# qdrvm/erasure-coding-crust

Hardware: AMD Instinct MI355X
Metric: device-resident encode+reconstruct GiB/s (and % HBM roofline), n_val=1024 (higher is better)
Workload: dtype u16

## Files before the change

### erasure-coding-crust_amd/csrc/capi.cpp

```cpp
#include <hip/hip_runtime.h>

#include <algorithm>
#include <chrono>
#include <cstdio>
#include <cstdlib>
#include <cstring>
#include <optional>
#include <string>
#include <vector>

#include "../../include/erasure_coding/ec_amd.h"
#include "../../include/erasure_coding/erasure_coding.h"
#include "ec_kernels.hpp"
#include "ec_runtime.hpp"
#include "gf_field.hpp"

using namespace ecamd;

namespace {

struct Workspace {
  void *ptr;
  size_t bytes;
};
// ... 568 lines not shown
                                      unsigned long slen, unsigned long sstride,
                                      const uint8_t *d_present, const uint16_t *d_err_log,
                                      unsigned long batch, uint8_t *d_out,
                                      unsigned long ostride, void *stream) {
  return ECCR_AMD_reconstruct_batch_patterns(nv, d_shards, slen, sstride, d_present, d_err_log,
                                             nullptr, batch, d_out, ostride, stream);
}

const char *ECCR_AMD_encode_kernel(unsigned long nv, const uint8_t *d_payloads, unsigned long plen,
                                   unsigned long pstride, unsigned long batch,
                                   const uint8_t *d_shards, unsigned long sstride) {
  CodeParams p;
  if (code_params(nv, &p) != ParamError::kOk || plen == 0) return nullptr;
  if (sstride < shard_len(p.k, plen) || pstride < plen) return nullptr;
  return kernel_name(choose_encode(p, plen, pstride, batch, reinterpret_cast<uintptr_t>(d_payloads),
                                   reinterpret_cast<uintptr_t>(d_shards), sstride));
}

const char *ECCR_AMD_reconstruct_kernel(unsigned long nv, const uint8_t *d_shards,
                                        unsigned long slen, unsigned long sstride,
                                        const uint8_t *d_present, const uint16_t *d_err_log,
                                        unsigned long batch, const uint8_t *d_out,
                                        unsigned long ostride) {
  CodeParams p;
  if (code_params(nv, &p) != ParamError::kOk || slen % 2 != 0) return nullptr;
  if (sstride < slen || ostride < slen * p.k) return nullptr;
  const ReconOverrides &o = recon_overrides();
  return kernel_name(choose_reconstruct(
      p, slen, sstride, batch, reinterpret_cast<uintptr_t>(d_shards),
      reinterpret_cast<uintptr_t>(d_present), reinterpret_cast<uintptr_t>(d_err_log),
      reinterpret_cast<uintptr_t>(d_out), ostride, o.waves8, o.force_packed));
}

NPRSResult ECCR_AMD_locator_cache_stats(unsigned long *hits, unsigned long *misses) {
  DeviceState *d = device_state();
  if (!d) return result(NPRS_RESULT_UNKNOWN_RECONSTRUCTION);
  locator_cache_stats(d, hits, misses);
  return result(NPRS_RESULT_OK);
}

NPRSResult ECCR_AMD_systematic_batch(unsigned long nv, const uint8_t *d_shards, unsigned long slen,
                                     unsigned long sstride, unsigned long batch, uint8_t *d_out,
                                     unsigned long ostride, void *stream) {
  CodeParams p;
  NPRSResult r = params_or_error(nv, &p);
  if (r.tag != NPRS_RESULT_OK) return r;
  if (sstride < slen || ostride < slen / 2 * 2 * p.k) return result(NPRS_RESULT_NON_UNIFORM_CHUNKS);
  if (!device_state()) return result(NPRS_RESULT_UNKNOWN_RECONSTRUCTION);
  if (!hip_check(launch_systematic(p, d_shards, slen / 2 * 2, sstride, batch, d_out, ostride,
                                   static_cast<hipStream_t>(stream)),
                 "systematic launch"))
    return result(NPRS_RESULT_UNKNOWN_RECONSTRUCTION);
  return result(NPRS_RESULT_OK);
}

void ECCR_AMD_set_scratch_limit(unsigned long bytes) { set_scratch_limit(bytes); }

int ECCR_AMD_release_stream_scratch(void *stream) {
  DeviceState *d = device_state();
  return d && release_stream_scratch(d, static_cast<hipStream_t>(stream)) ? 1 : 0;
}

const char *ECCR_AMD_last_error(void) { return last_error(); }

}
```

### erasure-coding-crust_amd/csrc/dec_n1024x.hip

```cpp
#include <hip/hip_runtime.h>

#include "dec_n1024_common.hpp"
#include "ec_device.hpp"
#include "ec_kernels.hpp"
#include "cimg.hpp"

namespace ecamd {
namespace {
using namespace n1024;
constexpr int WAVES = 12;
constexpr int THREADS = 64 * WAVES;
constexpr int COLS = 4 * WAVES;
constexpr int TAB_REGION = int(kCImgBytes);
static_assert(TAB_REGION % 8192 == 0, "regions 8 KB aligned: region addresses are base | rz");
constexpr uint32_t STG = uint32_t(TAB_REGION + WAVES * REG_BYTES);
constexpr uint32_t STG_PITCH = 112;
__device__ __forceinline__ uint32_t stg_row(uint32_t y) { return STG + (((y & 3) << 6) | (y >> 2)) * STG_PITCH; }
constexpr uint32_t SLOT = STG + 256 * STG_PITCH;
constexpr int LDS_BYTES = int(SLOT + 16);
static_assert(LDS_BYTES <= 160 * 1024, "LDS budget");
constexpr int ROW_WORDS = COLS / 2;

__host__ __device__ constexpr uint32_t rz(uint32_t v) {
  return ((v >> 5) << 8) | (((v ^ (v >> 4) ^ (v >> 5)) & 31) << 3);
}

__device__ __forceinline__ uint32_t posA2_reg(int r) { return uint32_t(r & 3) | (uint32_t(r >> 2) << 8); }
__device__ __forceinline__ uint32_t posB2_lane(uint32_t lane) { return (lane & 3) | ((lane >> 2) << 6); }
__device__ __forceinline__ uint32_t posC_reg(int r) {
  return (uint32_t((r >> 2) & 3) << 6) | (uint32_t(r & 3) << 8);
}

__device__ __forceinline__ void ipassA2(S16 &s, uint32_t lane) {
  const uint32_t l0 = cimg_lin(lane << 1), l1 = cimg_lin(lane);
  SubTab S0, S1;
  F9Tab F0, F1;
  Tab G0, G1;
  ctab(l0, cimg_lin(0), S0);
  ctab(l0, cimg_lin(1), S1);
  ctab(l0, cimg_lin(128), F0);
  ib(s, 0, 1, S0);
  ctab(l0, cimg_lin(129), F1);
  ib(s, 2, 3, S1);
  ctab(l0, cimg_lin(256), G0);
  ib(s, 4, 5, F0);
  ctab(l0, cimg_lin(257), G1);
  ib(s, 6, 7, F1);
  ib(s, 8, 9, G0);
  ctab(l0, cimg_lin(384), G0);
  ib(s, 10, 11, G1);
  ctab(l0, cimg_lin(385), G1);
  ctab(l1, cimg_lin(0), S0);
  ib(s, 12, 13, G0);
  ctab(l1, cimg_lin(64), S1);
// ... 42 lines not shown
  ctab(0u, cimg_lin(3), X3);
  ctab(0u, cimg_lin(4), X4);
  bx(s, 0, 4);
  ib(s, 8, 12, X1);
  ib(s, 1, 5, X2);
  ib(s, 9, 13, X3);
  ib(s, 2, 6, X4);
  ctab(0u, cimg_lin(5), X4);
  ib(s, 10, 14, X4);
  ctab(0u, cimg_lin(6), X4);
  ib(s, 3, 7, X4);
  ctab(0u, cimg_lin(7), X4);
  ib(s, 11, 15, X4);
  bx(s, 0, 8);
  bx(s, 4, 12);
  ib(s, 1, 9, X1);
  ib(s, 5, 13, X1);
  ib(s, 2, 10, X2);
  ib(s, 6, 14, X2);
  ib(s, 3, 11, X3);
  ib(s, 7, 15, X3);
#pragma unroll
  for (int q = 0; q < 4; ++q) {
    bx(s, 4 * q, 4 * q + 1);
    ib(s, 4 * q + 2, 4 * q + 3, X1);
  }
#pragma unroll
  for (int q = 0; q < 4; ++q) {
    bx(s, 4 * q, 4 * q + 2);
    bx(s, 4 * q + 1, 4 * q + 3);
  }
}

__device__ __forceinline__ void load_row_tail96(const uint8_t *row, uint32_t avail, uint32_t (&w)[ROW_WORDS]) {
  const uint32_t nw = (avail + 3) / 4;
  const uint32_t last = (avail & 3) ? (1u << (8 * (avail & 3))) - 1 : ~0u;
  const uint32_t *r = reinterpret_cast<const uint32_t *>(row);
#pragma unroll
  for (int j = 0; j < ROW_WORDS; ++j) {
    w[j] = 0;
    if (uint32_t(j) < nw) w[j] = r[j] & (uint32_t(j) + 1 == nw ? last : ~0u);
  }
}

}

__global__ void __launch_bounds__(THREADS) reconstruct_n1024x(
    const uint8_t *__restrict__ shards, uint64_t slen, uint64_t sstride,
    const uint8_t *__restrict__ present, const uint16_t *__restrict__ elog,
    const uint32_t *__restrict__ pattern, const uint32_t *__restrict__ order,
    uint8_t *__restrict__ out, uint64_t ostride, int nv, uint32_t batch, uint32_t *tick, DevTables t) {
  extern __shared__ __attribute__((aligned(16))) uint8_t lds[];
  uint8_t *regions = lds + TAB_REGION;
  volatile uint32_t *slot = reinterpret_cast<volatile uint32_t *>(lds + SLOT);
  const uint32_t tid0 = threadIdx.x, wave = tid0 >> 6;
  uint32_t taken = 0;
  if (tid0 == 0) taken = gridDim.x + atomicAdd(tick, 1u);
  uint8_t *my = regions + wave * REG_BYTES;

  {
    constexpr int kPer = (TAB_REGION / 16 + THREADS - 1) / THREADS;
    typedef uint32_t v4u __attribute__((ext_vector_type(4)));
    v4u v[kPer];
#pragma unroll
    for (int k = 0; k < kPer; ++k) {
      const uint32_t i = tid0 + k * THREADS;
      if (i < uint32_t(TAB_REGION / 16)) v[k] = reinterpret_cast<const v4u *>(t.cimg)[i];
    }
#pragma unroll
    for (int k = 0; k < kPer; ++k) {
      const uint32_t i = tid0 + k * THREADS;
      if (i < uint32_t(TAB_REGION / 16)) reinterpret_cast<v4u *>(lds)[i] = v[k];
    }
  }
  __syncthreads();
  if (tid0 == 0) *slot = taken;

  const uint64_t ncols = slen / 2;
  const uint32_t tiles_pp = uint32_t((ncols + COLS - 1) / COLS);
  const uint64_t total = uint64_t(tiles_pp) * batch;
  const uint32_t wave_s = __builtin_amdgcn_readfirstlane(tid0 >> 6);
  const auto load_meta = [&](uint64_t bw, uint32_t tid, uint32_t (&m)[4]) {
    const uint64_t pt = pattern ? pattern[bw] : bw;
    m[0] = order[bw * N + tid];
    m[1] = tid + THREADS < uint32_t(N) ? order[bw * N + THREADS + tid] : 0xFFFFu;
    const uint32_t y0 = 4 * (tid & 63);
    const uint32_t p4 = *reinterpret_cast<const uint32_t *>(present + pt * N + y0);
    const uint2 e4 = *reinterpret_cast<const uint2 *>(elog + pt * N + y0);
#pragma unroll
    for (int q = 0; q < 4; ++q) {
      const uint32_t e = ((q < 2 ? e4.x : e4.y) >> (16 * (q & 1))) & 0xFFFFu;
      const uint32_t f = ((p4 >> (8 * q)) & 0xFFu) ? 0xFFFFu : mul_index(e);
      if (q & 1) m[2 + (q >> 1)] |= f << 16;
      else m[2 + (q >> 1)] = f;
    }
  };
  uint32_t meta[4] = {0, 0, 0, 0}, meta_next[4] = {0, 0, 0, 0};
  uint32_t cur = blockIdx.x;
  if (cur < total) load_meta(cur / tiles_pp, tid0, meta);
  while (cur < total) {
    uint32_t tid = tid0;
    asm volatile("" : "+v"(tid));
    const uint32_t lane = tid & 63;
    const uint32_t bq = cur / tiles_pp;
    const uint64_t b = bq, col0 = uint64_t(cur - bq * tiles_pp) * COLS;
    const uint8_t *SH = shards + b * uint64_t(nv) * sstride;
    uint8_t *O = out + b * ostride;

    uint32_t nxt;
    {
      uint32_t w[ROW_WORDS] = {};
      Tab RT = {};
      const uint64_t avail = slen - 2 * col0;
      const auto load_row = [&](int half) __attribute__((always_inline)) {
        const uint8_t *row = SH + uint64_t(meta[half] >> 16) * sstride + 2 * col0;
        if (avail >= 2 * COLS) {
#pragma unroll
          for (int q = 0; q < ROW_WORDS / 4; ++q) {
            const uint4 d = reinterpret_cast<const uint4 *>(row)[q];
            w[4 * q] = d.x;
            w[4 * q + 1] = d.y;
            w[4 * q + 2] = d.z;
            w[4 * q + 3] = d.w;
          }
        } else {
          load_row_tail96(row, uint32_t(avail), w);
        }
        load_tab(t.mtab_tin, meta[half] & 0xffffu, RT);
      };
      if ((meta[0] & 0xffffu) != 0xffffu) load_row(0);
      lds_barrier();
      nxt = __builtin_amdgcn_readfirstlane(*slot);
      if (tid0 == 0) taken = gridDim.x + atomicAdd(tick, 1u);
#pragma unroll
      for (int half = 0; half < 2; ++half) {
        if (half == 1 && tid >= uint32_t(N - THREADS)) break;
        const uint32_t v = meta[half] >> 16;
        const bool on = (meta[half] & 0xffffu) != 0xffffu;
        if (half == 1 && on) load_row(1);
        uint32_t l[WAVES], h[WAVES];
#pragma unroll
        for (int g = 0; g < WAVES; ++g) l[g] = h[g] = 0;
        if (on) {
          if (v < uint32_t(K)) {
#pragma unroll
            for (int j = 0; j < ROW_WORDS / 4; ++j)
              *reinterpret_cast<__attribute__((address_space(3))) v4u *>(uintptr_t(stg_row(v) + 16 * j)) =
                  v4u{w[4 * j], w[4 * j + 1], w[4 * j + 2], w[4 * j + 3]};
          }
#pragma unroll
          for (int g = 0; g < WAVES; ++g) {
            const uint32_t a = w[2 * g], c = w[2 * g + 1];
            const uint32_t xh = vperm(c, a, 0x06040200u), xl = vperm(c, a, 0x07050301u);
            mul_acc(xl, xh, RT, l[g], h[g]);
          }
        }
#pragma unroll
        for (int g = 0; g < WAVES; ++g)
          *reinterpret_cast<uint2 *>(regions + g * REG_BYTES + rz(v)) = make_uint2(l[g], h[g]);
      }
    }
    if (nxt < total) load_meta(nxt / tiles_pp, tid, meta_next);
    __syncthreads();
    const uint64_t cbase = col0 + 4 * uint64_t(wave_s);
    if (cbase >= ncols) {
#pragma unroll
      for (int i = 0; i < 4; ++i) meta[i] = meta_next[i];
      cur = nxt;
      continue;
    }

    S16 s;
    {
      const uint32_t la = lds_addr(my) | rz(lane << 2);
#pragma unroll
      for (int r = 0; r < 16; ++r) {
        const uint2 x = lds_ld2(la ^ rz(posA2_reg(r)));
        s.l[r] = x.x;
        s.h[r] = x.y;
      }
      ipassA2(s, lane);
#pragma unroll
      for (int r = 0; r < 16; ++r) lds_st2(la ^ rz(posA2_reg(r)), make_uint2(s.l[r], s.h[r]));
      __builtin_amdgcn_fence(__ATOMIC_ACQ_REL, "wavefront");
      __builtin_amdgcn_wave_barrier();
    }
    {
      const uint32_t lb = lds_addr(my) | rz(posB2_lane(lane));
#pragma unroll
      for (int r = 0; r < 16; ++r) {
        const uint2 x = lds_ld2(lb ^ rz(uint32_t(r) << 2));
        s.l[r] = x.x;
        s.h[r] = x.y;
      }
      ipassB2(s, lane);
#pragma unroll
      for (int r = 0; r < 16; ++r) lds_st2(lb ^ rz(uint32_t(r) << 2), make_uint2(s.l[r], s.h[r]));
      __builtin_amdgcn_fence(__ATOMIC_ACQ_REL, "wavefront");
      __builtin_amdgcn_wave_barrier();
    }
    const uint32_t lc = lds_addr(my) | rz(lane);
#pragma unroll
    for (int r = 0; r < 16; ++r) {
      const uint2 x = lds_ld2(lc ^ rz(posC_reg(r)));
      s.l[r] = x.x;
      s.h[r] = x.y;
    }
    ipassC2(s);

    Tab T5[4];
#pragma unroll
    for (int q = 0; q < 4; ++q) {
      const uint32_t m = (meta[2 + (q >> 1)] >> (16 * (q & 1))) & 0xFFFFu;
      load_tab(t.mtab_tout, m != 0xFFFFu ? m : 0u, T5[q]);
    }

    uint32_t ql[4], qh[4];
    {
      const uint32_t keep0 = ((lane ^ (lane >> 1)) & 1) ? 0u : 0xffffffffu;
      const uint32_t m4 = ((lane >> 4) & 1) ? 0u : 0xffffffffu;
      const uint32_t m5 = ((lane >> 5) & 1) ? 0u : 0xffffffffu;
      const auto lane_terms = [&](uint32_t c0, uint32_t acc) {
        acc ^= uint32_t(__builtin_amdgcn_update_dpp(0, int(c0), 0xF5, 0xf, 0xf, false));
        acc ^= uint32_t(__builtin_amdgcn_update_dpp(0, int(c0), 0xEE, 0xf, 0xf, false));
        acc ^= uint32_t(__builtin_amdgcn_update_dpp(0, int(c0), 0x104, 0xf, 0x5, false));
        acc ^= uint32_t(__builtin_amdgcn_update_dpp(0, int(c0), 0x108, 0xf, 0x3, false));
        acc = __builtin_amdgcn_bitop3_b32(acc, from_upper(c0, 4), m4, 0x78);
        acc = __builtin_amdgcn_bitop3_b32(acc, from_upper(c0, 5), m5, 0x78);
        return __builtin_amdgcn_bitop3_b32(acc, c0, keep0, 0x78);
      };
#pragma unroll
      for (int q = 0; q < 4; ++q) {
        uint32_t al = s.l[4 * q + 1] ^ s.l[4 * q + 2], ah = s.h[4 * q + 1] ^ s.h[4 * q + 2];
        if (!(q & 1)) {
          al ^= s.l[4 * (q | 1)];
          ah ^= s.h[4 * (q | 1)];
        }
        if (!(q & 2)) {
          al ^= s.l[4 * (q | 2)];
          ah ^= s.h[4 * (q | 2)];
        }
        ql[q] = lane_terms(s.l[4 * q], al);
// ... 61 lines not shown
      swap_bit(qh[1], qh[3], 3, l3);
      fb(0, 2, T[0]);
      fb(1, 3, T[0]);
      ctab(0u, L(8), T[0]);
      fb(0, 1, T[1]);
      ctab(0u, L(9), T[1]);
      fb(2, 3, T[0]);
      ctab(0u, L(10), T[0]);
      const bool l0 = lane & 1, l1 = (lane >> 1) & 1;
      swap_bit(ql[0], ql[1], 0, l0);
      swap_bit(qh[0], qh[1], 0, l0);
      swap_bit(ql[2], ql[3], 0, l0);
      swap_bit(qh[2], qh[3], 0, l0);
      swap_bit(ql[0], ql[2], 1, l1);
      swap_bit(qh[0], qh[2], 1, l1);
      swap_bit(ql[1], ql[3], 1, l1);
      swap_bit(qh[1], qh[3], 1, l1);
      fb(0, 2, T[1]);
      fb(1, 3, T[1]);
      ctab(0u, L(11), T[1]);
      fb(0, 1, T[0]);
      fb(2, 3, T[1]);
    }

    {
      uint32_t ol[4], oh[4];
#pragma unroll
      for (int q = 0; q < 4; ++q) {
        const uint32_t m = (meta[2 + (q >> 1)] >> (16 * (q & 1))) & 0xFFFFu;
        ol[q] = oh[q] = 0;
        if (m != 0xFFFFu) {
          mul_acc(ql[q], qh[q], T5[q], ol[q], oh[q]);
        } else {
          const uint2 rv = lds_ld2(stg_row(4 * lane + uint32_t(q)) + 8 * wave_s);
          oh[q] = vperm(rv.y, rv.x, 0x06040200u);
          ol[q] = vperm(rv.y, rv.x, 0x07050301u);
        }
      }
#pragma unroll
      for (int c = 0; c < 4; ++c) {
        const uint64_t col = cbase + c;
        if (col >= ncols) break;
        const uint32_t w0 = vperm(ol[0], oh[0], 0x0c0c0400u + 0x0101u * c) |
                            (vperm(ol[1], oh[1], 0x0c0c0400u + 0x0101u * c) << 16);
        const uint32_t w1 = vperm(ol[2], oh[2], 0x0c0c0400u + 0x0101u * c) |
                            (vperm(ol[3], oh[3], 0x0c0c0400u + 0x0101u * c) << 16);
        *reinterpret_cast<uint2 *>(O + (col * K + 4 * lane) * 2) = make_uint2(w0, w1);
      }
    }
    if (tid0 == 0) *slot = taken;
#pragma unroll
    for (int i = 0; i < 4; ++i) meta[i] = meta_next[i];
    cur = nxt;
  }
}

size_t n1024_tick_offset(const CodeParams &p, size_t batch) { return (gather_order_bytes(p, batch) + 255) / 256 * 256; }
size_t n1024_scratch_bytes(const CodeParams &p, size_t batch) { return n1024_tick_offset(p, batch) + 256; }

static_assert(size_t(COLS) == kN1024xMinCols, "choose_reconstruct: at least one whole tile");

hipError_t launch_reconstruct_n1024x(const CodeParams &p, const DevTables &t,
                                     const uint8_t *d_shards, size_t slen, size_t sstride,
                                     const uint8_t *d_present, const uint16_t *d_err_log,
                                     const uint32_t *d_pattern, size_t batch, uint8_t *d_out,
                                     size_t ostride, void *scratch, hipStream_t s) {
  int cus = 0;
  if (!t.cimg || !scratch || slen / 2 < size_t(COLS)) return hipErrorInvalidValue;
  if (const hipError_t e = prepare_kernel(reinterpret_cast<const void *>(&reconstruct_n1024x), LDS_BYTES, &cus);
      e != hipSuccess)
    return e;
  const size_t tiles = (slen / 2 + COLS - 1) / COLS * batch;
  if (tiles + 4096 >= (size_t(1) << 32)) return hipErrorInvalidValue;
  uint32_t *order = static_cast<uint32_t *>(scratch);
  uint32_t *tick = reinterpret_cast<uint32_t *>(static_cast<uint8_t *>(scratch) + n1024_tick_offset(p, batch));
  if (const hipError_t e = launch_gather_order(p, d_present, d_err_log, d_pattern, batch, order, s);
      e != hipSuccess)
    return e;
  if (const hipError_t e = launch_zero_counters(tick, sizeof(uint32_t), s); e != hipSuccess) return e;
  const unsigned grid = unsigned(tiles < size_t(cus) ? tiles : size_t(cus));
  hipLaunchKernelGGL(reconstruct_n1024x, dim3(grid), dim3(THREADS), LDS_BYTES, s, d_shards, uint64_t(slen),
                     uint64_t(sstride), d_present, d_err_log, d_pattern, order, d_out, uint64_t(ostride),
                     int(p.nv), uint32_t(batch), tick, t);
  return hipGetLastError();
}

}
```

### erasure-coding-crust_amd/csrc/ec_kernels.hip

```cpp
#include <hip/hip_runtime.h>

#include <cstdlib>

#include "ec_device.hpp"
#include "ec_kernels.hpp"

namespace ecamd {
namespace {

constexpr int kBlock = 256;
constexpr int kLdsSlots = 4096;

__device__ __forceinline__ void ld(uint2 *p, uint32_t &l, uint32_t &h) {
  const uint2 v = *p;
  l = v.x;
  h = v.y;
}

constexpr int kPreStages = 3;
__device__ void ifft_g(uint2 *S, int logG, int logsz, uint32_t index, const DevTables t) {
  const int G = 1 << logG;
  const int half = (1 << logsz) >> 1;
  if (logsz <= kPreStages && half * G <= int(blockDim.x)) {
    const int b = threadIdx.x, g = b & (G - 1), pi = b >> logG;
// ... 609 lines not shown
  const size_t shm = size_t(p.n) * sizeof(uint16_t);
  int cus = 0;
  if (const hipError_t e = prepare_kernel(reinterpret_cast<const void *>(&error_locator_g), 65536 * 2, &cus);
      e != hipSuccess)
    return e;
  hipLaunchKernelGGL(error_locator_g, dim3(unsigned(batch)), dim3(kBlock), shm, s, d_present,
                     int(p.nv), ilog2(p.n), d_fold, d_pattern, d_err_log,
                     static_cast<uint16_t *>(nullptr));
  return hipGetLastError();
}

hipError_t launch_broadcast_locators(const CodeParams &p, const uint32_t *d_pattern, size_t batch,
                                     uint16_t *d_err_log, hipStream_t s) {
  if (batch == 0) return hipSuccess;
  hipLaunchKernelGGL(pattern_broadcast, dim3(unsigned(batch)), dim3(kBlock), 0, s, d_pattern,
                     int(p.n), d_err_log);
  return hipGetLastError();
}

size_t reconstruct_scratch_bytes(const CodeParams &p, size_t slen, size_t batch) {
  if (n4096_applicable(p)) return n4096_scratch_bytes(p, batch);
  if (n1024_applicable(p)) return n1024_scratch_bytes(p, batch);
  if (decgen_applicable(p)) return gather_order_bytes(p, batch);
  if (p.n <= uint32_t(kLdsSlots)) return 0;
  const size_t tiles = (slen / 2 + 3) / 4;
  return tiles * grid_y(batch) * 2 * size_t(p.n) * sizeof(uint2);
}

const ReconOverrides &recon_overrides() {
  static const ReconOverrides o = [] {
    const char *w = std::getenv("ECCR_AMD_RECON_WAVES"), *k = std::getenv("ECCR_AMD_RECON_PACKED");
    ReconOverrides r;
    r.waves8 = w && w[0] == '8';
    r.force_packed = k && k[0] == '1';
    return r;
  }();
  return o;
}

Kernel choose_reconstruct(const CodeParams &p, size_t slen, size_t sstride, size_t batch,
                          uintptr_t shards, uintptr_t present, uintptr_t err_log, uintptr_t out,
                          size_t ostride, bool waves8, bool force_packed) {
  if (batch == 0 || slen < 2) return Kernel::invalid;
  const bool aligned = shards % 16 == 0 && out % 8 == 0 && sstride % 16 == 0 &&
                       (batch == 1 || ostride % 8 == 0);
  const bool out8 = out % 8 == 0 && (batch == 1 || ostride % 8 == 0) && present % 16 == 0 &&
                    err_log % 16 == 0;
  const bool out16 = out % 16 == 0 && (batch == 1 || ostride % 16 == 0);
  const size_t ncols = slen / 2;
  if (n1024_applicable(p)) {
    const bool packed = ncols < kN1024Cols || shards % 16 != 0 || sstride % 16 != 0;
    if (!packed && aligned && out8 && !waves8 && ncols >= kN1024xMinCols) return Kernel::reconstruct_n1024x;
    if (packed ? out8 && shards % 2 == 0 && sstride % 2 == 0 : aligned && out8) {
      if (!packed && !force_packed) return Kernel::reconstruct_n1024;
      const size_t ncols4 = (ncols + 3) / 4 * 4;
      return ncols4 * batch + kN1024Cols < (size_t(1) << 32) ? Kernel::reconstruct_n1024_packed
                                                             : Kernel::invalid;
    }
  }
  if (aligned && out16 && n4096_applicable(p)) return Kernel::reconstruct_n4096;
  if (aligned && out16 && decgen_applicable(p)) return Kernel::reconstruct_gen;
  return Kernel::reconstruct_g;
}

hipError_t launch_reconstruct(const CodeParams &p, const DevTables &t, const uint8_t *d_shards,
                              size_t slen, size_t sstride, const uint8_t *d_present,
// ... 55 lines not shown
```

### erasure-coding-crust_amd/csrc/ec_kernels.hpp

```cpp
#pragma once

#include <hip/hip_runtime.h>

#include <cstddef>
#include <cstdint>

#include "gf_field.hpp"

namespace ecamd {

constexpr size_t kTabImageBytes = 5 * 1024 * 16;
constexpr int kTabImages = 4;

constexpr int tower_sub_min(int q) { return q == 0 ? 2 : q == 1 ? 3 : 4; }

constexpr int kF9Images = 2;
constexpr bool f9_slot(int kind, uint32_t i) {
  return i % 4 == 1 || (kind == 1 && i % 2 == 0 && i >= 256 && i < 512);
}

constexpr uint32_t kCImgGen = 0, kCImgGenPlane = 4096;
constexpr uint32_t kCImgF9 = 20480, kCImgF9Plane = 2048;
constexpr uint32_t kCImgSub0 = 28672, kCImgSub1 = 30720;
constexpr uint32_t kCImgBytes = 32768;
// ... 22 lines not shown

struct HostSig {
  uint32_t *flag = nullptr;
  uint32_t v = 0;
  bool fused = false;
};

hipError_t prepare_kernel(const void *fn, int lds_bytes, int *cus);

size_t encode_scratch_bytes(const CodeParams &p, size_t payload_len, size_t batch);
bool encode_scratch_optional(const CodeParams &p);
size_t reconstruct_scratch_bytes(const CodeParams &p, size_t shard_len, size_t batch);

enum class Kernel {
  invalid,
  encode_k256w,
  encode_k256_packed,
  encode_kw,
  encode_k512w,
  encode_k1024,
  encode_g,
  reconstruct_n1024x,
  reconstruct_n1024,
  reconstruct_n1024_packed,
  reconstruct_n4096,
  reconstruct_gen,
  reconstruct_g,
};
const char *kernel_name(Kernel k);

Kernel choose_encode(const CodeParams &p, size_t payload_len, size_t payload_stride, size_t batch,
                     uintptr_t payloads, uintptr_t shards, size_t shard_stride);
struct ReconOverrides {
  bool waves8 = false, force_packed = false;
};
const ReconOverrides &recon_overrides();
Kernel choose_reconstruct(const CodeParams &p, size_t shard_len, size_t shard_stride, size_t batch,
                          uintptr_t shards, uintptr_t present, uintptr_t err_log, uintptr_t out,
                          size_t out_stride, bool waves8, bool force_packed);

hipError_t launch_encode(const CodeParams &p, const DevTables &t, const uint8_t *d_payloads,
                         size_t payload_len, size_t payload_stride, size_t batch, uint8_t *d_shards,
                         size_t shard_stride, void *scratch, hipStream_t s, HostSig *sig = nullptr);

hipError_t launch_error_locator(const CodeParams &p, const uint8_t *d_present, size_t batch,
                                const uint16_t *d_fold, const uint32_t *d_pattern,
                                uint16_t *d_err_log, hipStream_t s);
bool locator_wave_applicable(uint32_t n);
hipError_t launch_signal_host(uint32_t *h_flag, uint32_t v, hipStream_t s);
hipError_t launch_zero_counters(uint32_t *p, size_t bytes, hipStream_t s);
size_t dedup_scratch_bytes(size_t batch);
hipError_t launch_dedup_patterns(const CodeParams &p, const uint8_t *d_present, size_t batch,
                                 uint32_t *d_pattern, void *scratch, hipStream_t s);
hipError_t launch_broadcast_locators(const CodeParams &p, const uint32_t *d_pattern, size_t batch,
                                     uint16_t *d_err_log, hipStream_t s);

hipError_t launch_reconstruct(const CodeParams &p, const DevTables &t, const uint8_t *d_shards,
                              size_t shard_len, size_t shard_stride, const uint8_t *d_present,
                              const uint16_t *d_err_log, const uint32_t *d_pattern, size_t batch,
                              uint8_t *d_out, size_t out_stride, void *scratch, hipStream_t s);

hipError_t launch_systematic(const CodeParams &p, const uint8_t *d_shards, size_t shard_len,
                             size_t shard_stride, size_t batch, uint8_t *d_out, size_t out_stride,
                             hipStream_t s, HostSig *sig = nullptr);

constexpr int kTinyMaxN = 16;
constexpr size_t kTinyBytes = 2048;
bool tiny_applicable(const CodeParams &p, size_t plen, size_t ostride);
hipError_t launch_encode_tiny(const CodeParams &p, const DevTables &t, const uint8_t *h_payload, size_t plen,
                              uint8_t *out, size_t ostride, hipStream_t s, HostSig *sig);
bool systematic_tiny_applicable(const CodeParams &p, size_t slen);
hipError_t launch_systematic_tiny(const CodeParams &p, const uint8_t *h_shards, size_t slen, size_t sstride,
                                  uint8_t *out, hipStream_t s, HostSig *sig);
hipError_t warm_encode_tiny(hipStream_t s);

bool k256_applicable(const CodeParams &p);
constexpr size_t kK256Tile = 128, kN1024Cols = 32, kN1024xMinCols = 48;
hipError_t launch_encode_k256(const CodeParams &p, const DevTables &t, const uint8_t *d_payloads,
                              size_t plen, size_t pstride, size_t batch, uint8_t *d_shards,
                              size_t sstride, hipStream_t s);
size_t k256_scratch_bytes(const CodeParams &p);
hipError_t launch_encode_k256w(const CodeParams &p, const DevTables &t, const uint8_t *d_payloads,
                               size_t plen, size_t pstride, size_t batch, uint8_t *d_shards,
                               size_t sstride, void *scratch, hipStream_t s);

bool k1024_applicable(const CodeParams &p);
size_t k1024_scratch_bytes(size_t plen, size_t batch);
hipError_t launch_encode_k1024(const CodeParams &p, const DevTables &t, const uint8_t *d_payloads,
                               size_t plen, size_t pstride, size_t batch, uint8_t *d_shards,
                               size_t sstride, void *scratch, hipStream_t s);

bool k512w_applicable(const CodeParams &p);
size_t k512w_scratch_bytes(const CodeParams &p);
hipError_t launch_encode_k512w(const CodeParams &p, const DevTables &t, const uint8_t *d_payloads,
                               size_t plen, size_t pstride, size_t batch, uint8_t *d_shards,
                               size_t sstride, void *scratch, hipStream_t s);

bool kw_applicable(const CodeParams &p);
size_t kw_scratch_bytes(const CodeParams &p);
hipError_t launch_encode_kw(const CodeParams &p, const DevTables &t, const uint8_t *d_payloads,
                            size_t plen, size_t pstride, size_t batch, uint8_t *d_shards,
                            size_t sstride, void *scratch, hipStream_t s);

size_t gather_order_bytes(const CodeParams &p, size_t batch);
hipError_t launch_gather_order(const CodeParams &p, const uint8_t *d_present,
                               const uint16_t *d_err_log, const uint32_t *d_pattern, size_t batch,
                               uint32_t *order, hipStream_t s);

bool n1024_applicable(const CodeParams &p);
hipError_t launch_reconstruct_n1024(const CodeParams &p, const DevTables &t, bool packed,
                                    const uint8_t *d_shards, size_t slen, size_t sstride,
                                    const uint8_t *d_present, const uint16_t *d_err_log,
                                    const uint32_t *d_pattern, size_t batch, uint8_t *d_out,
                                    size_t ostride, void *scratch, hipStream_t s);
size_t n1024_scratch_bytes(const CodeParams &p, size_t batch);
size_t n1024_tick_offset(const CodeParams &p, size_t batch);
hipError_t launch_reconstruct_n1024x(const CodeParams &p, const DevTables &t,
                                     const uint8_t *d_shards, size_t slen, size_t sstride,
                                     const uint8_t *d_present, const uint16_t *d_err_log,
                                     const uint32_t *d_pattern, size_t batch, uint8_t *d_out,
                                     size_t ostride, void *scratch, hipStream_t s);

bool n4096_applicable(const CodeParams &p);
size_t n4096_scratch_bytes(const CodeParams &p, size_t batch);
hipError_t launch_reconstruct_n4096(const CodeParams &p, const DevTables &t,
                                    const uint8_t *d_shards, size_t slen, size_t sstride,
                                    const uint8_t *d_present, const uint16_t *d_err_log,
                                    const uint32_t *d_pattern, size_t batch, uint8_t *d_out,
                                    size_t ostride, void *scratch, hipStream_t s);

bool decgen_applicable(const CodeParams &p);
hipError_t launch_reconstruct_gen(const CodeParams &p, const DevTables &t,
                                  const uint8_t *d_shards, size_t slen, size_t sstride,
                                  const uint8_t *d_present, const uint16_t *d_err_log,
                                  const uint32_t *d_pattern, size_t batch, uint8_t *d_out,
                                  size_t ostride, void *scratch, hipStream_t s);

}
```

### erasure-coding-crust_amd/ecc_amd.py

```python
from __future__ import annotations

import ctypes as C
import enum
import os
import subprocess

try:
    import torch
except Exception:
    torch = None

HERE = os.path.dirname(os.path.abspath(__file__))
LIB_PATH = os.environ.get("ECC_AMD_LIB") or os.path.join(HERE, "lib", "liberasure_coding_crust.so")
HEADERS = [os.path.join(os.path.dirname(HERE), "include", "erasure_coding", h)
           for h in ("erasure_coding.h", "ec_amd.h")]


class Tag(enum.IntEnum):
    OK = 0
    TOO_MANY_VALIDATORS = 1
    NOT_ENOUGH_VALIDATORS = 2
    WRONG_VALIDATOR_COUNT = 3
    NOT_ENOUGH_CHUNKS = 4
    TOO_MANY_CHUNKS = 5
# ... 53 lines not shown

def lib():
    global _lib
    if _lib is None:
        if not os.path.exists(LIB_PATH):
            build()
        L = C.CDLL(LIB_PATH)
        ul, up, vp = C.c_ulong, C.POINTER(C.c_ulong), C.c_void_p
        sig = {
            "ECCR_get_recovery_threshold": (NPRSResult, [ul, up]),
            "ECCR_deallocate_data_block": (None, [C.POINTER(DataBlock)]),
            "ECCR_deallocate_chunk": (None, [C.POINTER(Chunk)]),
            "ECCR_deallocate_chunk_list": (None, [C.POINTER(ChunksList)]),
            "ECCR_AFFT_Table": (NPRSResult, [C.POINTER(C.c_uint16 * 65535)]),
            "ECCR_Test_MeasurePerformance": (NPRSResult, [C.POINTER(DataBlock), ul, up, up]),
            "ECCR_obtain_chunks": (NPRSResult, [ul, C.POINTER(DataBlock), C.POINTER(ChunksList)]),
            "ECCR_reconstruct_from_systematic": (NPRSResult, [ul, C.POINTER(ChunksList),
                                                              C.POINTER(DataBlock)]),
            "ECCR_reconstruct": (NPRSResult, [ul, C.POINTER(ChunksList), C.POINTER(DataBlock)]),
            "ECCR_AMD_code_params": (NPRSResult, [ul, up, up, up]),
            "ECCR_AMD_shard_len": (ul, [ul, ul]),
            "ECCR_AMD_device_count": (C.c_int, []),
            "ECCR_AMD_init_device": (NPRSResult, []),
            "ECCR_AMD_encode_batch": (NPRSResult, [ul, vp, ul, ul, ul, vp, ul, vp]),
            "ECCR_AMD_error_locator": (NPRSResult, [ul, vp, ul, vp, vp]),
            "ECCR_AMD_reconstruct_batch": (NPRSResult, [ul, vp, ul, ul, vp, vp, ul, vp, ul, vp]),
            "ECCR_AMD_systematic_batch": (NPRSResult, [ul, vp, ul, ul, ul, vp, ul, vp]),
            "ECCR_AMD_dedup_patterns": (NPRSResult, [ul, vp, ul, vp, vp]),
            "ECCR_AMD_error_locator_patterns": (NPRSResult, [ul, vp, vp, ul, vp, vp]),
            "ECCR_AMD_reconstruct_batch_patterns": (NPRSResult, [ul, vp, ul, ul, vp, vp, vp, ul, vp,
                                                                 ul, vp]),
            "ECCR_AMD_encode_kernel": (C.c_char_p, [ul, vp, ul, ul, ul, vp, ul]),
            "ECCR_AMD_reconstruct_kernel": (C.c_char_p, [ul, vp, ul, ul, vp, vp, ul, vp, ul]),
            "ECCR_AMD_locator_cache_stats": (NPRSResult, [up, up]),
            "ECCR_AMD_encode_workspace_bytes": (ul, [ul, ul, ul]),
            "ECCR_AMD_error_locator_workspace_bytes": (ul, [ul, ul]),
            "ECCR_AMD_reconstruct_workspace_bytes": (ul, [ul, ul, ul]),
            "ECCR_AMD_encode_batch_ws": (NPRSResult, [ul, vp, ul, ul, ul, vp, ul, vp, ul, vp]),
            "ECCR_AMD_error_locator_ws": (NPRSResult, [ul, vp, ul, vp, vp, ul, vp]),
            "ECCR_AMD_reconstruct_batch_ws": (NPRSResult, [ul, vp, ul, ul, vp, vp, vp, ul, vp, ul,
                                                           vp, ul, vp]),
            "ECCR_AMD_host_alloc": (vp, [ul]),
            "ECCR_AMD_host_free": (None, [vp]),
            "ECCR_AMD_encode_host_batch": (NPRSResult, [ul, vp, ul, ul, ul, vp, ul, ul]),
            "ECCR_AMD_reconstruct_host_batch": (NPRSResult, [ul, vp, ul, ul, vp, ul, ul, vp, ul,
                                                             ul]),
            "ECCR_AMD_set_scratch_limit": (None, [ul]),
            "ECCR_AMD_release_stream_scratch": (C.c_int, [vp]),
            "ECCR_AMD_last_error": (C.c_char_p, []),
        }
        for name, (res, args) in sig.items():
            try:
                f = getattr(L, name)
            except AttributeError:
                if os.environ.get("ECC_AMD_LIB"):
                    continue
                raise
            f.restype = res
            f.argtypes = args
        _lib = L
    return _lib


def _check(res: NPRSResult, where: str):
    if res.tag != Tag.OK:
        raise ECError(res, where)
# ... 177 lines not shown
                                          _p(d_shards), shard_stride, wp, wb, _stream(stream)),
           "encode_batch_ws")


def error_locator_ws(nv, d_present, batch, d_err_log, ws, stream=None):
    wp, wb = _ws(ws)
    _check(lib().ECCR_AMD_error_locator_ws(nv, _p(d_present), batch, _p(d_err_log), wp, wb,
                                           _stream(stream)), "error_locator_ws")


def reconstruct_batch_ws(nv, d_shards, shard_len_, shard_stride, d_present, d_err_log, batch,
                         d_out, out_stride, ws, d_pattern=None, stream=None):
    wp, wb = _ws(ws)
    _check(lib().ECCR_AMD_reconstruct_batch_ws(
        nv, _p(d_shards), shard_len_, shard_stride, _p(d_present), _p(d_err_log),
        None if d_pattern is None else _p(d_pattern), batch, _p(d_out), out_stride, wp, wb,
        _stream(stream)), "reconstruct_batch_ws")


def encode_kernel(nv, d_payloads, payload_len, payload_stride, batch, d_shards, shard_stride):
    r = lib().ECCR_AMD_encode_kernel(nv, _p(d_payloads), payload_len, payload_stride, batch,
                                     _p(d_shards), shard_stride)
    return None if r is None else r.decode()


def reconstruct_kernel(nv, d_shards, shard_len_, shard_stride, d_present, d_err_log, batch, d_out,
                       out_stride):
    r = lib().ECCR_AMD_reconstruct_kernel(nv, _p(d_shards), shard_len_, shard_stride,
                                          _p(d_present), _p(d_err_log), batch, _p(d_out),
                                          out_stride)
    return None if r is None else r.decode()


def locator_cache_stats():
    h, m = C.c_ulong(), C.c_ulong()
    _check(lib().ECCR_AMD_locator_cache_stats(C.byref(h), C.byref(m)), "locator_cache_stats")
    return h.value, m.value


def systematic_batch(nv, d_shards, shard_len_, shard_stride, batch, d_out, out_stride, stream=None):
    _check(lib().ECCR_AMD_systematic_batch(nv, _p(d_shards), shard_len_, shard_stride, batch,
                                           _p(d_out), out_stride, _stream(stream)),
           "systematic_batch")




def encode_host_batch(nv, h_payloads, payload_len, payload_stride, batch, h_shards, shard_stride,
                      chunk=0):
    _check(lib().ECCR_AMD_encode_host_batch(nv, _p(h_payloads), payload_len, payload_stride,
                                            batch, _p(h_shards), shard_stride, chunk),
           "encode_host_batch")


def reconstruct_host_batch(nv, h_shards, shard_len_, shard_stride, h_index, count, batch, h_out,
                           out_stride, chunk=0):
    _check(lib().ECCR_AMD_reconstruct_host_batch(nv, _p(h_shards), shard_len_, shard_stride,
                                                 _p(h_index), count, batch, _p(h_out), out_stride,
                                                 chunk),
           "reconstruct_host_batch")
```

### include/erasure_coding/ec_amd.h

```cpp
#ifndef ERASURE_CODING_EC_AMD_H_
#define ERASURE_CODING_EC_AMD_H_

#include "erasure_coding.h"

#ifdef __cplusplus
extern "C" {
#endif

struct NPRSResult ECCR_AMD_code_params(unsigned long n_validators, unsigned long *n,
                                       unsigned long *k, unsigned long *threshold);

unsigned long ECCR_AMD_shard_len(unsigned long n_validators, unsigned long payload_len);

int ECCR_AMD_device_count(void);

struct NPRSResult ECCR_AMD_init_device(void);

struct NPRSResult ECCR_AMD_encode_batch(unsigned long n_validators, const uint8_t *d_payloads,
                                        unsigned long payload_len, unsigned long payload_stride,
                                        unsigned long batch, uint8_t *d_shards,
                                        unsigned long shard_stride, void *stream);

struct NPRSResult ECCR_AMD_error_locator(unsigned long n_validators, const uint8_t *d_present,
                                         unsigned long batch, uint16_t *d_err_log,
// ... 20 lines not shown
                                            unsigned long batch, uint16_t *d_err_log,
                                            void *d_workspace, unsigned long workspace_bytes,
                                            void *stream);
struct NPRSResult ECCR_AMD_reconstruct_batch_ws(
    unsigned long n_validators, const uint8_t *d_shards, unsigned long shard_len,
    unsigned long shard_stride, const uint8_t *d_present, const uint16_t *d_err_log,
    const uint32_t *d_pattern, unsigned long batch, uint8_t *d_out, unsigned long out_stride,
    void *d_workspace, unsigned long workspace_bytes, void *stream);


struct NPRSResult ECCR_AMD_dedup_patterns(unsigned long n_validators, const uint8_t *d_present,
                                          unsigned long batch, uint32_t *d_pattern, void *stream);

struct NPRSResult ECCR_AMD_error_locator_patterns(unsigned long n_validators,
                                                  const uint8_t *d_present,
                                                  const uint32_t *d_pattern, unsigned long batch,
                                                  uint16_t *d_err_log, void *stream);

struct NPRSResult ECCR_AMD_reconstruct_batch_patterns(
    unsigned long n_validators, const uint8_t *d_shards, unsigned long shard_len,
    unsigned long shard_stride, const uint8_t *d_present, const uint16_t *d_err_log,
    const uint32_t *d_pattern, unsigned long batch, uint8_t *d_out, unsigned long out_stride,
    void *stream);

const char *ECCR_AMD_encode_kernel(unsigned long n_validators, const uint8_t *d_payloads,
                                   unsigned long payload_len, unsigned long payload_stride,
                                   unsigned long batch, const uint8_t *d_shards,
                                   unsigned long shard_stride);
const char *ECCR_AMD_reconstruct_kernel(unsigned long n_validators, const uint8_t *d_shards,
                                        unsigned long shard_len, unsigned long shard_stride,
                                        const uint8_t *d_present, const uint16_t *d_err_log,
                                        unsigned long batch, const uint8_t *d_out,
                                        unsigned long out_stride);

struct NPRSResult ECCR_AMD_locator_cache_stats(unsigned long *hits, unsigned long *misses);

struct NPRSResult ECCR_AMD_systematic_batch(unsigned long n_validators, const uint8_t *d_shards,
                                            unsigned long shard_len, unsigned long shard_stride,
                                            unsigned long batch, uint8_t *d_out,
                                            unsigned long out_stride, void *stream);

void *ECCR_AMD_host_alloc(unsigned long bytes);
void ECCR_AMD_host_free(void *ptr);

struct NPRSResult ECCR_AMD_encode_host_batch(unsigned long n_validators, const uint8_t *h_payloads,
                                             unsigned long payload_len,
                                             unsigned long payload_stride, unsigned long batch,
                                             uint8_t *h_shards, unsigned long shard_stride,
                                             unsigned long chunk);

struct NPRSResult ECCR_AMD_reconstruct_host_batch(unsigned long n_validators,
                                                  const uint8_t *h_shards, unsigned long shard_len,
                                                  unsigned long shard_stride,
                                                  const uint16_t *h_index, unsigned long count,
                                                  unsigned long batch, uint8_t *h_out,
                                                  unsigned long out_stride, unsigned long chunk);

void ECCR_AMD_set_scratch_limit(unsigned long bytes);

int ECCR_AMD_release_stream_scratch(void *stream);

const char *ECCR_AMD_last_error(void);

#ifdef __cplusplus
}
#endif
// ... 3 lines not shown
```

Baseline: 231.7.

## Add 16-wave n1024x reconstruct variant that reads passthrough rows from global memory

Templates the n1024x reconstruct kernel on wave count and adds a 16-wave form. It is selected by default when the shard is wide enough, with an env override to force 12 waves. The 16-wave form drops the LDS staging area for systematic rows and instead reloads rows marked present straight from global memory before the output pass. This trades extra global reads for more waves per workgroup, wider tiles and less LDS use.

```diff
diff --git a/erasure-coding-crust_amd/csrc/capi.cpp b/erasure-coding-crust_amd/csrc/capi.cpp
--- a/erasure-coding-crust_amd/csrc/capi.cpp
+++ b/erasure-coding-crust_amd/csrc/capi.cpp
@@ -624,6 +624,8 @@
       reinterpret_cast<uintptr_t>(d_out), ostride, o.waves8, o.force_packed));
 }
 
+int ECCR_AMD_reconstruct_n1024x_waves(unsigned long slen) { return n1024x_waves(slen); }
+
 NPRSResult ECCR_AMD_locator_cache_stats(unsigned long *hits, unsigned long *misses) {
   DeviceState *d = device_state();
   if (!d) return result(NPRS_RESULT_UNKNOWN_RECONSTRUCTION);
diff --git a/erasure-coding-crust_amd/csrc/dec_n1024x.hip b/erasure-coding-crust_amd/csrc/dec_n1024x.hip
--- a/erasure-coding-crust_amd/csrc/dec_n1024x.hip
+++ b/erasure-coding-crust_amd/csrc/dec_n1024x.hip
@@ -8,18 +8,26 @@
 namespace ecamd {
 namespace {
 using namespace n1024;
-constexpr int WAVES = 12;
-constexpr int THREADS = 64 * WAVES;
-constexpr int COLS = 4 * WAVES;
 constexpr int TAB_REGION = int(kCImgBytes);
 static_assert(TAB_REGION % 8192 == 0, "regions 8 KB aligned: region addresses are base | rz");
-constexpr uint32_t STG = uint32_t(TAB_REGION + WAVES * REG_BYTES);
 constexpr uint32_t STG_PITCH = 112;
-__device__ __forceinline__ uint32_t stg_row(uint32_t y) { return STG + (((y & 3) << 6) | (y >> 2)) * STG_PITCH; }
-constexpr uint32_t SLOT = STG + 256 * STG_PITCH;
-constexpr int LDS_BYTES = int(SLOT + 16);
-static_assert(LDS_BYTES <= 160 * 1024, "LDS budget");
-constexpr int ROW_WORDS = COLS / 2;
+template <int WAVES>
+struct Form {
+  static_assert(WAVES == 12 || WAVES == 16, "three or four waves per SIMD");
+  static constexpr int THREADS = 64 * WAVES;
+  static constexpr int COLS = 4 * WAVES;
+  static constexpr int ROW_WORDS = COLS / 2;
+  static constexpr int SLOTS = (N + THREADS - 1) / THREADS;
+  static constexpr bool STAGED = WAVES == 12;
+  static constexpr uint32_t STG = uint32_t(TAB_REGION + WAVES * REG_BYTES);
+  static constexpr uint32_t SLOT = STAGED ? STG + 256 * STG_PITCH : kCImgSub1 + 4;
+  static constexpr int LDS_BYTES = STAGED ? int(SLOT + 16) : int(STG);
+  static_assert(LDS_BYTES <= 160 * 1024, "LDS budget");
+};
+template <int WAVES>
+__device__ __forceinline__ uint32_t stg_row(uint32_t y) {
+  return Form<WAVES>::STG + (((y & 3) << 6) | (y >> 2)) * STG_PITCH;
+}
 
 __host__ __device__ constexpr uint32_t rz(uint32_t v) {
   return ((v >> 5) << 8) | (((v ^ (v >> 4) ^ (v >> 5)) & 31) << 3);
@@ -128,7 +136,8 @@
   }
 }
 
-__device__ __forceinline__ void load_row_tail96(const uint8_t *row, uint32_t avail, uint32_t (&w)[ROW_WORDS]) {
+template <int ROW_WORDS>
+__device__ __forceinline__ void load_row_tail(const uint8_t *row, uint32_t avail, uint32_t (&w)[ROW_WORDS]) {
   const uint32_t nw = (avail + 3) / 4;
   const uint32_t last = (avail & 3) ? (1u << (8 * (avail & 3))) - 1 : ~0u;
   const uint32_t *r = reinterpret_cast<const uint32_t *>(row);
@@ -141,11 +150,15 @@
 
 }
 
-__global__ void __launch_bounds__(THREADS) reconstruct_n1024x(
+template <int WAVES>
+__global__ void __launch_bounds__(64 * WAVES) reconstruct_n1024x(
     const uint8_t *__restrict__ shards, uint64_t slen, uint64_t sstride,
     const uint8_t *__restrict__ present, const uint16_t *__restrict__ elog,
     const uint32_t *__restrict__ pattern, const uint32_t *__restrict__ order,
     uint8_t *__restrict__ out, uint64_t ostride, int nv, uint32_t batch, uint32_t *tick, DevTables t) {
+  using F = Form<WAVES>;
+  constexpr int THREADS = F::THREADS, COLS = F::COLS, ROW_WORDS = F::ROW_WORDS;
+  constexpr uint32_t SLOT = F::SLOT;
   extern __shared__ __attribute__((aligned(16))) uint8_t lds[];
   uint8_t *regions = lds + TAB_REGION;
   volatile uint32_t *slot = reinterpret_cast<volatile uint32_t *>(lds + SLOT);
@@ -179,7 +192,7 @@
   const auto load_meta = [&](uint64_t bw, uint32_t tid, uint32_t (&m)[4]) {
     const uint64_t pt = pattern ? pattern[bw] : bw;
     m[0] = order[bw * N + tid];
-    m[1] = tid + THREADS < uint32_t(N) ? order[bw * N + THREADS + tid] : 0xFFFFu;
+    if constexpr (F::SLOTS == 2) m[1] = tid + THREADS < uint32_t(N) ? order[bw * N + THREADS + tid] : 0xFFFFu;
     const uint32_t y0 = 4 * (tid & 63);
     const uint32_t p4 = *reinterpret_cast<const uint32_t *>(present + pt * N + y0);
     const uint2 e4 = *reinterpret_cast<const uint2 *>(elog + pt * N + y0);
@@ -220,7 +233,7 @@
             w[4 * q + 3] = d.w;
           }
         } else {
-          load_row_tail96(row, uint32_t(avail), w);
+          load_row_tail<ROW_WORDS>(row, uint32_t(avail), w);
         }
         load_tab(t.mtab_tin, meta[half] & 0xffffu, RT);
       };
@@ -229,7 +242,7 @@
       nxt = __builtin_amdgcn_readfirstlane(*slot);
       if (tid0 == 0) taken = gridDim.x + atomicAdd(tick, 1u);
 #pragma unroll
-      for (int half = 0; half < 2; ++half) {
+      for (int half = 0; half < F::SLOTS; ++half) {
         if (half == 1 && tid >= uint32_t(N - THREADS)) break;
         const uint32_t v = meta[half] >> 16;
         const bool on = (meta[half] & 0xffffu) != 0xffffu;
@@ -238,11 +251,13 @@
 #pragma unroll
         for (int g = 0; g < WAVES; ++g) l[g] = h[g] = 0;
         if (on) {
-          if (v < uint32_t(K)) {
-#pragma unroll
-            for (int j = 0; j < ROW_WORDS / 4; ++j)
-              *reinterpret_cast<__attribute__((address_space(3))) v4u *>(uintptr_t(stg_row(v) + 16 * j)) =
-                  v4u{w[4 * j], w[4 * j + 1], w[4 * j + 2], w[4 * j + 3]};
+          if constexpr (F::STAGED) {
+            if (v < uint32_t(K)) {
+#pragma unroll
+              for (int j = 0; j < ROW_WORDS / 4; ++j)
+                *reinterpret_cast<__attribute__((address_space(3))) v4u *>(uintptr_t(stg_row<WAVES>(v) + 16 * j)) =
+                    v4u{w[4 * j], w[4 * j + 1], w[4 * j + 2], w[4 * j + 3]};
+            }
           }
 #pragma unroll
           for (int g = 0; g < WAVES; ++g) {
@@ -304,6 +319,16 @@
     }
     ipassC2(s);
 
+    uint2 RV[4];
+#pragma unroll
+    for (int q = 0; q < 4; ++q) {
+      const uint32_t m = (meta[2 + (q >> 1)] >> (16 * (q & 1))) & 0xFFFFu;
+      RV[q] = make_uint2(0, 0);
+      if constexpr (!F::STAGED) {
+        if (m == 0xFFFFu)
+          RV[q] = *reinterpret_cast<const uint2 *>(SH + uint64_t(4 * lane + uint32_t(q)) * sstride + 2 * cbase);
+      }
+    }
     Tab T5[4];
 #pragma unroll
     for (int q = 0; q < 4; ++q) {
@@ -431,7 +456,8 @@
         if (m != 0xFFFFu) {
           mul_acc(ql[q], qh[q], T5[q], ol[q], oh[q]);
         } else {
-          const uint2 rv = lds_ld2(stg_row(4 * lane + uint32_t(q)) + 8 * wave_s);
+          uint2 rv = RV[q];
+          if constexpr (F::STAGED) rv = lds_ld2(stg_row<WAVES>(4 * lane + uint32_t(q)) + 8 * wave_s);
           oh[q] = vperm(rv.y, rv.x, 0x06040200u);
           ol[q] = vperm(rv.y, rv.x, 0x07050301u);
         }
@@ -457,19 +483,26 @@
 size_t n1024_tick_offset(const CodeParams &p, size_t batch) { return (gather_order_bytes(p, batch) + 255) / 256 * 256; }
 size_t n1024_scratch_bytes(const CodeParams &p, size_t batch) { return n1024_tick_offset(p, batch) + 256; }
 
-static_assert(size_t(COLS) == kN1024xMinCols, "choose_reconstruct: at least one whole tile");
-
-hipError_t launch_reconstruct_n1024x(const CodeParams &p, const DevTables &t,
-                                     const uint8_t *d_shards, size_t slen, size_t sstride,
-                                     const uint8_t *d_present, const uint16_t *d_err_log,
-                                     const uint32_t *d_pattern, size_t batch, uint8_t *d_out,
-                                     size_t ostride, void *scratch, hipStream_t s) {
+static_assert(size_t(Form<12>::COLS) == kN1024xMinCols, "choose_reconstruct: at least one whole tile");
+static_assert(size_t(Form<16>::COLS) <= kN1024x16MinCols, "n1024x_waves: at least one whole tile");
+
+int n1024x_waves(size_t slen) {
+  return !recon_overrides().waves12 && slen / 2 >= kN1024x16MinCols ? 16 : 12;
+}
+
+namespace {
+template <int WAVES>
+hipError_t launch_form(const CodeParams &p, const DevTables &t, const uint8_t *d_shards, size_t slen,
+                       size_t sstride, const uint8_t *d_present, const uint16_t *d_err_log,
+                       const uint32_t *d_pattern, size_t batch, uint8_t *d_out, size_t ostride,
+                       void *scratch, hipStream_t s) {
+  using F = Form<WAVES>;
   int cus = 0;
-  if (!t.cimg || !scratch || slen / 2 < size_t(COLS)) return hipErrorInvalidValue;
-  if (const hipError_t e = prepare_kernel(reinterpret_cast<const void *>(&reconstruct_n1024x), LDS_BYTES, &cus);
+  if (!t.cimg || !scratch || slen / 2 < size_t(F::COLS)) return hipErrorInvalidValue;
+  if (const hipError_t e = prepare_kernel(reinterpret_cast<const void *>(&reconstruct_n1024x<WAVES>), F::LDS_BYTES, &cus);
       e != hipSuccess)
     return e;
-  const size_t tiles = (slen / 2 + COLS - 1) / COLS * batch;
+  const size_t tiles = (slen / 2 + F::COLS - 1) / F::COLS * batch;
   if (tiles + 4096 >= (size_t(1) << 32)) return hipErrorInvalidValue;
   uint32_t *order = static_cast<uint32_t *>(scratch);
   uint32_t *tick = reinterpret_cast<uint32_t *>(static_cast<uint8_t *>(scratch) + n1024_tick_offset(p, batch));
@@ -478,10 +511,23 @@
     return e;
   if (const hipError_t e = launch_zero_counters(tick, sizeof(uint32_t), s); e != hipSuccess) return e;
   const unsigned grid = unsigned(tiles < size_t(cus) ? tiles : size_t(cus));
-  hipLaunchKernelGGL(reconstruct_n1024x, dim3(grid), dim3(THREADS), LDS_BYTES, s, d_shards, uint64_t(slen),
-                     uint64_t(sstride), d_present, d_err_log, d_pattern, order, d_out, uint64_t(ostride),
-                     int(p.nv), uint32_t(batch), tick, t);
+  hipLaunchKernelGGL(reconstruct_n1024x<WAVES>, dim3(grid), dim3(F::THREADS), F::LDS_BYTES, s, d_shards,
+                     uint64_t(slen), uint64_t(sstride), d_present, d_err_log, d_pattern, order, d_out,
+                     uint64_t(ostride), int(p.nv), uint32_t(batch), tick, t);
   return hipGetLastError();
 }
-
-}
+}
+
+hipError_t launch_reconstruct_n1024x(const CodeParams &p, const DevTables &t,
+                                     const uint8_t *d_shards, size_t slen, size_t sstride,
+                                     const uint8_t *d_present, const uint16_t *d_err_log,
+                                     const uint32_t *d_pattern, size_t batch, uint8_t *d_out,
+                                     size_t ostride, void *scratch, hipStream_t s) {
+  return n1024x_waves(slen) == 16
+             ? launch_form<16>(p, t, d_shards, slen, sstride, d_present, d_err_log, d_pattern, batch, d_out,
+                               ostride, scratch, s)
+             : launch_form<12>(p, t, d_shards, slen, sstride, d_present, d_err_log, d_pattern, batch, d_out,
+                               ostride, scratch, s);
+}
+
+}
diff --git a/erasure-coding-crust_amd/csrc/ec_kernels.hip b/erasure-coding-crust_amd/csrc/ec_kernels.hip
--- a/erasure-coding-crust_amd/csrc/ec_kernels.hip
+++ b/erasure-coding-crust_amd/csrc/ec_kernels.hip
@@ -665,6 +665,7 @@
     const char *w = std::getenv("ECCR_AMD_RECON_WAVES"), *k = std::getenv("ECCR_AMD_RECON_PACKED");
     ReconOverrides r;
     r.waves8 = w && w[0] == '8';
+    r.waves12 = w && w[0] == '1' && w[1] == '2';
     r.force_packed = k && k[0] == '1';
     return r;
   }();
diff --git a/erasure-coding-crust_amd/csrc/ec_kernels.hpp b/erasure-coding-crust_amd/csrc/ec_kernels.hpp
--- a/erasure-coding-crust_amd/csrc/ec_kernels.hpp
+++ b/erasure-coding-crust_amd/csrc/ec_kernels.hpp
@@ -78,7 +78,7 @@
 Kernel choose_encode(const CodeParams &p, size_t payload_len, size_t payload_stride, size_t batch,
                      uintptr_t payloads, uintptr_t shards, size_t shard_stride);
 struct ReconOverrides {
-  bool waves8 = false, force_packed = false;
+  bool waves8 = false, waves12 = false, force_packed = false;
 };
 const ReconOverrides &recon_overrides();
 Kernel choose_reconstruct(const CodeParams &p, size_t shard_len, size_t shard_stride, size_t batch,
@@ -121,7 +121,7 @@
 hipError_t warm_encode_tiny(hipStream_t s);
 
 bool k256_applicable(const CodeParams &p);
-constexpr size_t kK256Tile = 128, kN1024Cols = 32, kN1024xMinCols = 48;
+constexpr size_t kK256Tile = 128, kN1024Cols = 32, kN1024xMinCols = 48, kN1024x16MinCols = 145;
 hipError_t launch_encode_k256(const CodeParams &p, const DevTables &t, const uint8_t *d_payloads,
                               size_t plen, size_t pstride, size_t batch, uint8_t *d_shards,
                               size_t sstride, hipStream_t s);
@@ -159,6 +159,7 @@
                                     const uint8_t *d_present, const uint16_t *d_err_log,
                                     const uint32_t *d_pattern, size_t batch, uint8_t *d_out,
                                     size_t ostride, void *scratch, hipStream_t s);
+int n1024x_waves(size_t slen);
 size_t n1024_scratch_bytes(const CodeParams &p, size_t batch);
 size_t n1024_tick_offset(const CodeParams &p, size_t batch);
 hipError_t launch_reconstruct_n1024x(const CodeParams &p, const DevTables &t,
diff --git a/erasure-coding-crust_amd/ecc_amd.py b/erasure-coding-crust_amd/ecc_amd.py
--- a/erasure-coding-crust_amd/ecc_amd.py
+++ b/erasure-coding-crust_amd/ecc_amd.py
@@ -109,6 +109,7 @@
                                                                  ul, vp]),
             "ECCR_AMD_encode_kernel": (C.c_char_p, [ul, vp, ul, ul, ul, vp, ul]),
             "ECCR_AMD_reconstruct_kernel": (C.c_char_p, [ul, vp, ul, ul, vp, vp, ul, vp, ul]),
+            "ECCR_AMD_reconstruct_n1024x_waves": (C.c_int, [ul]),
             "ECCR_AMD_locator_cache_stats": (NPRSResult, [up, up]),
             "ECCR_AMD_encode_workspace_bytes": (ul, [ul, ul, ul]),
             "ECCR_AMD_error_locator_workspace_bytes": (ul, [ul, ul]),
@@ -352,6 +353,10 @@
     return None if r is None else r.decode()
 
 
+def reconstruct_n1024x_waves(shard_len_: int) -> int:
+    return int(lib().ECCR_AMD_reconstruct_n1024x_waves(shard_len_))
+
+
 def locator_cache_stats():
     h, m = C.c_ulong(), C.c_ulong()
     _check(lib().ECCR_AMD_locator_cache_stats(C.byref(h), C.byref(m)), "locator_cache_stats")
diff --git a/include/erasure_coding/ec_amd.h b/include/erasure_coding/ec_amd.h
--- a/include/erasure_coding/ec_amd.h
+++ b/include/erasure_coding/ec_amd.h
@@ -76,6 +76,7 @@
                                         const uint8_t *d_present, const uint16_t *d_err_log,
                                         unsigned long batch, const uint8_t *d_out,
                                         unsigned long out_stride);
+int ECCR_AMD_reconstruct_n1024x_waves(unsigned long shard_len);
 
 struct NPRSResult ECCR_AMD_locator_cache_stats(unsigned long *hits, unsigned long *misses);
 
```

Result: faster. 240.7, median of 6 (+3.9%).
